# glennhickey/teHmm

Hardware: AMD Instinct MI355X
Metric: genome positions/sec (Viterbi+posterior), 35 states x 10 tracks (higher is better)
Workload: dtype f64

## Files before the change

tehmm_amd/csrc/tehmm_fused.hip.h:

```cpp
#pragma once
#include "tehmm_lane.hip.h"

namespace tehmm {

template <int NT>
struct FusedGeom {
  static constexpr int KS = NT / 4;
  static constexpr int KSP = ((KS + 1) + 1) & ~1;
  static constexpr int RT = (NT + 15) / 16;
  static constexpr int SLICE_B = KSP * 8;
  static constexpr int ROW_D = 4 * KSP;
  static constexpr int ROW_D_LDS = 4 * KSP + 2;
};

#ifndef TEHMM_FUSED_2W
#define TEHMM_FUSED_2W 36
#endif
#define TEHMM_FUSED_BLKW 24
#ifndef TEHMM_FUSED_NSLOT_CAP
#define TEHMM_FUSED_NSLOT_CAP 64
#endif

struct FusedTab {
  const unsigned long long *rixx;
// ... 42 lines not shown
}
__device__ __forceinline__ double item_max4(double t) {
  const unsigned lo = __double2loint(t), hi = __double2hiint(t);
  const auto a = __builtin_amdgcn_permlane32_swap(lo, lo, false, false);
  const auto b = __builtin_amdgcn_permlane32_swap(hi, hi, false, false);
  const double t1 = fmax(__hiloint2double((int)b[0], (int)a[0]), __hiloint2double((int)b[1], (int)a[1]));
  const unsigned lo1 = __double2loint(t1), hi1 = __double2hiint(t1);
  const auto c = __builtin_amdgcn_permlane16_swap(lo1, lo1, false, false);
  const auto d = __builtin_amdgcn_permlane16_swap(hi1, hi1, false, false);
  return fmax(__hiloint2double((int)d[0], (int)c[0]), __hiloint2double((int)d[1], (int)c[1]));
}

typedef unsigned int fused_u4 __attribute__((ext_vector_type(4)));
struct IndexWindow {
  const fused_u4 *src;
  unsigned lds_base;
  int lane, dir, NB;
  int cur = -1;
  fused_u4 r0, r1, r2;
  bool inflight = false;

  __device__ __forceinline__ void request(int blk) {
    if (blk < 0 || blk >= NB) { inflight = false; return; }
    const fused_u4 *p = src + (int64_t)blk * 192 + lane * 3;
    r0 = p[0];
    r1 = p[1];
    r2 = p[2];
    inflight = true;
  }
  __device__ __forceinline__ void commit(int blk) {
    typedef __attribute__((address_space(3))) fused_u4 lds_u4;
    lds_u4 *d = (lds_u4 *)(size_t)(lds_base + (unsigned)((blk & 1) * 3072 + lane * 48));
    d[0] = r0;
    d[1] = r1;
    d[2] = r2;
    cur = blk;
  }
  __device__ __forceinline__ void start(int blk) {
    request(blk);
    commit(blk);
    request(blk + dir);
  }
  __device__ __forceinline__ void need(int blk) {
    if (blk != cur) {
      commit(blk);
      request(blk + dir);
    }
  }
  __device__ __forceinline__ unsigned word_addr(int blk, int r, int FKW, int w) const {
    return lds_base + (unsigned)((blk & 1) * 3072 + ((r * FKW + w) * 16 + (lane & 15)) * 8);
  }
};
__device__ __forceinline__ unsigned long long lds_read_u64(unsigned addr) {
  typedef __attribute__((address_space(3))) const unsigned long long lds_cu64;
  return *(lds_cu64 *)(size_t)addr;
}

template <int NT, bool LOGDOM>
struct EmisStream {
  using G = FusedGeom<NT>;
  static constexpr int NSLOT = G::KS < TEHMM_FUSED_NSLOT_CAP ? G::KS : TEHMM_FUSED_NSLOT_CAP;
  static constexpr int NGS = NSLOT > 1 ? 2 : 1;
  static constexpr int GF = NSLOT >= 8 ? 4 : NSLOT / 2;
  const FusedTab &ft;
  const double *lds;
  IndexWindow &win;
  const int kq;
  unsigned wbase = 0;
  double q[G::KS];
  double sc = 0.0;
  double xa[G::KSP];
  double xc[G::KSP];
  unsigned long long wcur = 0;

  __device__ __forceinline__ EmisStream(const FusedTab &ft_, const double *lds_, IndexWindow &win_, int kq_)
      : ft(ft_), lds(lds_), win(win_), kq(kq_) {}
  static __device__ __forceinline__ int entry(unsigned long long w, int i) { return (int)((w >> (16 * (i & 3))) & 0xffffull); }
  __device__ __forceinline__ unsigned long long word(int w) const { return lds_read_u64(wbase + (unsigned)w * 128u); }
  __device__ __forceinline__ void fold(const double (&x)[G::KSP]) {
#pragma unroll
    for (int s = 0; s < G::KS; ++s) q[s] = LOGDOM ? q[s] + x[s] : q[s] * x[s];
    if (!LOGDOM) sc += x[G::KS];
  }
  __device__ __forceinline__ void glb_request(int i) { fused_load_glb<NT>(ft.ptab, entry(word(i >> 2), i), kq, xa); }
  __device__ __forceinline__ void begin(int e) {
    const int blk = e / ft.SB, r = e - blk * ft.SB;
    win.need(blk);
    wbase = win.word_addr(blk, r, ft.FKW, 0);
#pragma unroll
    for (int s = 0; s < G::KS; ++s) q[s] = LOGDOM ? 0.0 : 1.0;
    sc = 0.0;
    glb_request(0);
    wcur = word(ft.n_glb >> 2);
  }
  __device__ __forceinline__ void slot(int k) {
    if (k >= NSLOT) return;
    const int il = ft.n_glb + k;
    if (k > 0) fold(xc);
    if (k == GF && NSLOT > 1) {
      fold(xa);
      glb_request(1);
    }
    fused_load_lds<NT>(lds, entry(wcur, il), kq, xc);
    if (k + 1 < NSLOT) wcur = word((il + 1) >> 2);
  }
  __device__ __forceinline__ void finish(int N, double (&qo)[G::KS], double &ms) {
    fold(xc);
    fold(xa);
    for (int i = NGS; i < ft.n_glb; ++i) {
      glb_request(i);
      fold(xa);
    }
    for (int il = ft.n_glb + NSLOT; il < ft.K; ++il) {
      fused_load_lds<NT>(lds, entry(word(il >> 2), il), kq, xc);
      fold(xc);
    }
    if (LOGDOM) {
      double m = -INFINITY;
#pragma unroll
      for (int s = 0; s < G::KS; ++s) {
        q[s] *= ft.normalize;
        m = fmax(m, kq + 4 * s < N ? q[s] : -INFINITY);
      }
      m = item_max4(m);
      const bool good = m > -1e20;
#pragma unroll
      for (int s = 0; s < G::KS; ++s) qo[s] = (good && kq + 4 * s < N) ? exp_nonpos(q[s] - m) : 0.0;
      ms = good ? m : 0.0;
    } else {
#pragma unroll
      for (int s = 0; s < G::KS; ++s) qo[s] = q[s];
      ms = sc;
    }
  }
};

template <int NT>
__host__ __device__ inline size_t fused_lds_bytes(int lds_rows, bool post_tiles) {
  return (size_t)lds_rows * FusedGeom<NT>::ROW_D_LDS * 8 + 4 * 2 * 3072 + (post_tiles ? 4 * (16 * NT * 8 + 128) : 0);
}
template <int NT>
__device__ __forceinline__ void fused_stage(const FusedTab &ft, double *lds) {
  const int n = ft.lds_rows * FusedGeom<NT>::ROW_D_LDS;
  for (int i = threadIdx.x; i < n; i += blockDim.x) lds[i] = ft.ptab_lds[i];
}

struct FusedOrder {
  int K, n_glb, FKW, KP, SB, NB, Wu;
  int zero_glb, zero_lds;
  unsigned char order[TEHMM_MAX_TRACKS];
  int base[TEHMM_MAX_TRACKS];
  int cnt[TEHMM_MAX_TRACKS];
};
__global__ __launch_bounds__(256) void k_fused_rowindex(IntervalTab iv, LaneGeom lg, FusedOrder fo, const uint8_t *obs,
                                                        unsigned long long *rixx) {
  const int E = fo.NB * fo.SB;
  const int64_t n = (int64_t)lg.n_groups * 4 * E * 16;
  const int per_blk = 16 * fo.SB;
  for (int64_t idx = blockIdx.x * (int64_t)blockDim.x + threadIdx.x; idx < n; idx += (int64_t)gridDim.x * blockDim.x) {
    const int64_t tb = idx / per_blk;
    const int rem = (int)(idx - tb * per_blk);
    const int i16 = rem / fo.SB;
    const int e = (int)(tb % fo.NB) * fo.SB + (rem - i16 * fo.SB);
    const int64_t tile = tb / fo.NB;
    const int64_t item = tile * 16 + i16;
    const bool valid = item < lg.n_items;
    const int id = valid ? lg.item_iv[item] : 0;
    const int64_t T = iv.len[id];
    int64_t t = (valid ? lg.item_t0[item] : 0) - fo.Wu + e;
    t = t < 0 ? 0 : (t >= T ? T - 1 : t);
    const uint8_t *orow = obs + (iv.pos0[id] + (T > 0 ? t : 0)) * fo.KP;
    const int blk = e / fo.SB, r = e - blk * fo.SB;
    unsigned long long *dst = rixx + ((tile * fo.NB + blk) * TEHMM_FUSED_BLKW + (int64_t)r * fo.FKW) * 16 + i16;
    for (int w = 0; w < fo.FKW; ++w) {
      unsigned long long word = 0;
      for (int b = 0; b < 4; ++b) {
        const int i = 4 * w + b;
        int v = 0;
        if (i < fo.K) {
          const int sym = orow[fo.order[i]];
          v = sym < fo.cnt[i] ? fo.base[i] + sym : (i < fo.n_glb ? fo.zero_glb : fo.zero_lds);
        }
        word |= (unsigned long long)(v & 0xffff) << (16 * b);
      }
      dst[(int64_t)w * 16] = word;
    }
  }
}

template <int NT, bool LOGDOM>
__global__ __launch_bounds__(256) __attribute__((amdgpu_waves_per_eu(NT <= TEHMM_FUSED_2W ? 2 : 1, NT <= TEHMM_FUSED_2W ? 2 : 1)))
void k_fused_fwd(IntervalTab iv, FusedTab ft, LaneGeom lg, int N, int CS, int Wu,
                 const double *__restrict__ tab , float *al32, double *chkf, double *pre,
                 double *end, double *slog32) {
  using G = FusedGeom<NT>;
  constexpr int KS = G::KS, RT = G::RT;
  extern __shared__ double fused_lds[];
  fused_stage<NT>(ft, fused_lds);
  __syncthreads();
  const int lane = threadIdx.x & 63;
  const int tile = blockIdx.x * 4 + (threadIdx.x >> 6);
  if (tile >= lg.n_groups * 4) return;
  const int L = lg.L;
  const int kq = lane >> 4;
  const int64_t item = (int64_t)tile * 16 + (lane & 15);
  const bool valid = item < lg.n_items;
  const int id = valid ? lg.item_iv[item] : 0;
  const int64_t t0 = valid ? lg.item_t0[item] : 0;
  const int64_t T = iv.len[id];
  const int64_t ct0 = (t0 / CS) * CS;
  const bool run = valid && ct0 + CS <= T && ct0 > 0;
  if (!__any(run)) return;
  double tf[RT][KS];
#pragma unroll
  for (int rt = 0; rt < RT; ++rt) {
#pragma unroll
    for (int s = 0; s < KS; ++s) {
      const int j = 16 * rt + (lane & 15), k = 4 * s + kq;
      tf[rt][s] = (j < NT) ? tab[k * NT + j] : 0.0;
    }
  }
  double v[KS];
#pragma unroll
  for (int s = 0; s < KS; ++s) v[s] = (kq + 4 * s < N) ? 1.0 / (double)N : 0.0;
  double slog = 0.0;
  auto vec_out = [&](double *dst) {
    const int64_t po = ((((item >> 6) * NT) + kq) << 6) + (item & 63);
#pragma unroll
    for (int s = 0; s < KS; ++s) dst[po + ((int64_t)(4 * s) << 6)] = v[s];
  };
  const double qnan = __longlong_as_double(0x7ff8000000000000LL);
  IndexWindow win;
  win.src = (const fused_u4 *)ft.rixx + (int64_t)tile * ft.NB * 192;
  win.lds_base = (unsigned)(size_t)(__attribute__((address_space(3))) const double *)fused_lds +
                 (unsigned)(ft.lds_rows * G::ROW_D_LDS * 8 + (threadIdx.x >> 6) * 2 * 3072);
  win.lane = lane;
  win.dir = 1;
  win.NB = ft.NB;
  win.start(0);
  double q[KS], ms;
  EmisStream<NT, LOGDOM> es(ft, fused_lds, win, kq);
  es.begin(0);
#pragma unroll
  for (int k = 0; k < KS; ++k) es.slot(k);
  es.finish(N, q, ms);
  const int E1 = ft.NB * ft.SB - 1;
  es.begin(min(1, E1));
  {
    float2 *ar = (float2 *)al32 + al32_index<NT>(lg, item, 0, kq) / 2;
#pragma unroll
    for (int p = 0; p < (KS + 1) / 2; ++p) ar[(int64_t)p * 64] = make_float2(0.f, 0.f);
  }
#ifdef TEHMM_STAMPS
  unsigned long long stq[4] = {0, 0, 0, 0}, stt = stamp_now();
#define FST(i) do { const unsigned long long n_ = stamp_now(); stq[i] += n_ - stt; stt = n_; } while (0)
#else
#define FST(i)
#endif
  for (int s = -Wu; s < L; ++s) {
    if (s == 0) {
      if (run) vec_out(pre);
      slog = 0.0;
    }
    FST(3);
    lane_d4 acc[RT];
#pragma unroll
    for (int rt = 0; rt < RT; ++rt) acc[rt] = (lane_d4){0.0, 0.0, 0.0, 0.0};
#pragma unroll
    for (int k = 0; k < KS; ++k) {
#pragma unroll
      for (int rt = 0; rt < RT; ++rt) acc[rt] = __builtin_amdgcn_mfma_f64_16x16x4f64(tf[rt][k], v[k], acc[rt], 0, 0, 0);
      es.slot(k);
      __builtin_amdgcn_sched_barrier(0);
    }
    FST(0);
    double qn[KS], msn = 0.0;
    es.finish(N, qn, msn);
    FST(1);
    double a[KS];
    double t = 0.0;
#pragma unroll
    for (int k = 0; k < KS; ++k) {
      a[k] = acc[k >> 2][k & 3] * q[k];
      t += a[k];
    }
    t = item_sum4(t);
    const int e = ((__double2hiint(t) >> 20) & 0x7ff) - 1022;
    const bool okrow = t > 1e-280 && t < INFINITY;
    const double scale = okrow ? __hiloint2double((1023 - e) << 20, 0) : qnan;
#pragma unroll
    for (int k = 0; k < KS; ++k) v[k] = a[k] * scale;
    slog += (double)e * 0.6931471805599453 + ms;
#pragma unroll
    for (int k = 0; k < KS; ++k) q[k] = qn[k];
    const double ms_now = ms;
    ms = msn;
    (void)ms_now;
    es.begin(min(s + 2 + Wu, E1));
    FST(2);
    {
      float2 *ar = (float2 *)al32 + al32_index<NT>(lg, item, s < 0 ? 0 : s, kq) / 2;
#pragma unroll
      for (int p = 0; p < (KS + 1) / 2; ++p)
        ar[(int64_t)p * 64] = run ? make_float2((float)v[2 * p], 2 * p + 1 < KS ? (float)v[2 * p + 1] : 0.f)
                                  : make_float2(0.f, 0.f);
    }
    if (s >= 0 && run) {
      if ((s & 31) == 31) {
        if (kq == 0) slog32[item * (L / 32) + (s >> 5)] = slog;
        if ((s & 63) == 31) {
          double *cr = chkf + (item * (L / 64) + (s >> 6)) * NT + kq;
#pragma unroll
          for (int k = 0; k < KS; ++k) cr[4 * k] = v[k];
        }
      }
    }
  }
  if (run) vec_out(end);
#ifdef TEHMM_STAMPS
  if (lane == 0 && blockIdx.x < 4096)
    for (int i = 0; i < 4; ++i) g_stamps[(blockIdx.x * 4 + (threadIdx.x >> 6)) * 4 + i] = stq[i];
#endif
#undef FST
}

template <int NT, bool LOGDOM, bool EPS, bool ESTEP = false>
__global__ __launch_bounds__(256) __attribute__((amdgpu_waves_per_eu(NT <= TEHMM_FUSED_2W ? 2 : 1, NT <= TEHMM_FUSED_2W ? 2 : 1)))
void k_fused_bwd(IntervalTab iv, FusedTab ft, LaneGeom lg, int N, int CS, int Wu,
                 const double *__restrict__ tab , const float *__restrict__ al32,
                 double *post, double *pre, double *end, double *chk, float *gam32 = nullptr, float *wz32 = nullptr,
                 double *sink = nullptr ) {
  using G = FusedGeom<NT>;
  constexpr int KS = G::KS, RT = G::RT;
  extern __shared__ double fused_lds[];
  fused_stage<NT>(ft, fused_lds);
  __syncthreads();
  const int lane = threadIdx.x & 63;
  const int tile = blockIdx.x * 4 + (threadIdx.x >> 6);
  if (tile >= lg.n_groups * 4) return;
// ... 201 lines not shown
```

tehmm_amd/csrc/tehmm_hip.hip:

```cpp
#include <climits>
#include "tehmm_kernels.hip.h"
#include "tehmm_coop.hip.h"
#include "tehmm_lane.hip.h"
#include "tehmm_lane3.hip.h"
#include "tehmm_place.hip.h"
#include "tehmm_aux.hip.h"
#include "tehmm_fused.hip.h"
#include "tehmm_estep.hip.h"
#include "tehmm_wide_estep.hip.h"
#include "tehmm_wide.hip.h"
#include "tehmm_large.hip.h"
#include "tehmm_map.hip.h"

#include <algorithm>
#include <atomic>
#include <cmath>
#include <cstdio>
#include <cstdlib>
#include <cstring>
#include <mutex>
#include <numeric>
#include <string>
#include <thread>
#include <vector>
// ... 1555 lines not shown
  return TEHMM_OK;
}

template <int NT>
static void launch_vit_stitch(tehmm_batch *b, const tehmm_model *m, const IntervalTab &iv, const VitChunks &vc,
                              hipStream_t st) {
  LaneWork &lw = b->lw;
  hipLaunchKernelGGL((k_vit_stitch<NT>), dim3((vc.n + 3) / 4), dim3(256), 0, st, iv, lane_geom(lw), vc,
                     lane_vit_items(lw), m->N, lw.soft_ties);
  hipLaunchKernelGGL((k_vit_links<NT>), dim3((vc.n + 3) / 4), dim3(256), 0, st, iv, lane_geom(lw), vc,
                     lane_vit_items(lw), m->N);
  hipLaunchKernelGGL(k_vit_runs, dim3(std::max(1, b->n)), dim3(64), 0, st, vc, b->n);
}

static LaneGeom lane_geom(const LaneWork &lw) {
  LaneGeom lg;
  lg.item_iv = lw.item_iv.p; lg.item_t0 = lw.item_t0.p; lg.ifirst = lw.ifirst.p;
  lg.n_items = lw.n_items; lg.n_groups = lw.n_groups; lg.L = lw.L;
  return lg;
}

template <int NT>
static void launch_emis_lane(tehmm_batch *b, const tehmm_model *m, const IntervalTab &iv, const EmisTab &em,
                             bool want_log, bool want_lin, bool want_f32, hipStream_t st) {
  LaneWork &lw = b->lw;
  const size_t lds = (size_t)em.lds_rows * NT * sizeof(double);
  allow_lds(k_emis_lane<NT>, lds);
  hipLaunchKernelGGL((k_emis_lane<NT>), dim3((lw.n_groups + 3) / 4), dim3(256), lds, st, iv, em, lane_geom(lw),
                     m->N, want_log ? lw.B.p : (double *)nullptr, want_lin ? lw.BH.p : (double *)nullptr, lw.MS.p,
                     want_f32 ? lw.B32.p : (float *)nullptr);
}

template <int NT>
static void launch_emis_gain_lane(tehmm_batch *b, const tehmm_model *m, const IntervalTab &iv, const EmisTab &em,
                                  int CS, int Wu, bool ratio, int emis_split, hipStream_t st) {
  LaneWork &lw = b->lw;
  if constexpr (NT >= 12) {
    const bool split = emis_split >= 0 ? emis_split != 0 : lw.n_groups < 2048;
    if (split) {
      constexpr int NW = TEHMM_P2_NW, NU = 2;
      const size_t lds3 = Emis3Geom<NT, NW, NU>::lds_bytes(em.lds_rows);
      const dim3 grid3((lw.n_groups + NU - 1) / NU);
      if constexpr (NT <= TEHMM_RATIO_LANE_MAX) if (ratio) {
        allow_lds(k_emis_gain_lane3<NT, NW, NU, true>, lds3);
        hipLaunchKernelGGL((k_emis_gain_lane3<NT, NW, NU, true>), grid3, dim3(64 * NW * NU), lds3, st, iv, em, lane_geom(lw),
                           m->N, CS, Wu, (const float *)m->ltP.p, lw.B.p, lw.vgain.p, (const double *)b->ratios.p);
        return;
      }
      allow_lds(k_emis_gain_lane3<NT, NW, NU, false>, lds3);
      hipLaunchKernelGGL((k_emis_gain_lane3<NT, NW, NU, false>), grid3, dim3(64 * NW * NU), lds3, st, iv, em, lane_geom(lw),
                         m->N, CS, Wu, (const float *)m->ltP.p, lw.B.p, lw.vgain.p, (const double *)nullptr);
      return;
    }
  }
  const size_t lds = (size_t)em.lds_rows * NT * sizeof(double);
  if constexpr (NT <= TEHMM_RATIO_LANE_MAX) if (ratio) {
    allow_lds(k_emis_gain_lane<NT, true>, lds);
    hipLaunchKernelGGL((k_emis_gain_lane<NT, true>), dim3((lw.n_groups + 3) / 4), dim3(256), lds, st, iv, em,
                       lane_geom(lw), m->N, CS, Wu, (const float *)m->ltP.p, lw.B.p, lw.vgain.p,
                       (const double *)b->ratios.p);
    return;
  }
  allow_lds(k_emis_gain_lane<NT>, lds);
  hipLaunchKernelGGL((k_emis_gain_lane<NT>), dim3((lw.n_groups + 3) / 4), dim3(256), lds, st, iv, em, lane_geom(lw),
                     m->N, CS, Wu, (const float *)m->ltP.p, lw.B.p, lw.vgain.p, (const double *)nullptr);
}

template <int NT>
static void launch_gain_lane(tehmm_batch *b, const tehmm_model *m, const IntervalTab &iv, int CS, int Wu,
                             hipStream_t st) {
  LaneWork &lw = b->lw;
  hipLaunchKernelGGL((k_vit_gain_lane<NT>), dim3((lw.n_groups + 3) / 4), dim3(256), 0, st, iv, lane_geom(lw), m->N,
                     CS, Wu, (const float *)m->ltP.p, (const float *)lw.B32.p, lw.vgain.p);
}

template <int NT>
static void launch_fb_lane(tehmm_batch *b, const tehmm_model *m, const IntervalTab &iv, const EmisTab &em_in,
                           const FbChunks &fc, int Wu, hipStream_t st, hipEvent_t ev_mid) {
  LaneWork &lw = b->lw;
  const LaneGeom lg = lane_geom(lw);
  const dim3 grid((lw.n_groups + 3) / 4);
  const dim3 gridc((fc.n + 255) / 256);
  const dim3 gridit((lw.n_items + 255) / 256);
  const dim3 gridi(std::max(1, b->n));
  const EmisTab em = b->n > 256 ? without_lds_tables(em_in) : em_in;
  size_t lds = ((size_t)2 * 64 * (NT + 1) + 2 * 64 + NT + (size_t)em.lds_rows * NT + 8) * sizeof(double);
  allow_lds(k_fb_fix<NT, 0, false, true>, lds);
  allow_lds(k_fb_fix<NT, 1, false, true>, lds);
  hipStream_t sS = b->sB;
  hipLaunchKernelGGL((k_fb_lane<NT, 0>), grid, dim3(256), 0, st, iv, lg, m->N, fc.CS, Wu, m->AG.p, lw.BH.p,
                     lw.MS.p, lw.AL.p, lw.pre_f.p, lw.end_f.p, lw.slog32.p);
  (void)hipEventRecord(b->evX[0], st);
  (void)hipStreamWaitEvent(sS, b->evX[0], 0);
  hipLaunchKernelGGL((k_fb_itemlinks<NT>), gridit, dim3(256), 0, sS, lg, m->N, lw.pre_f.p, lw.end_f.p, lw.pre_b.p,
                     lw.end_b.p, lw.dl_f.p, lw.lr_f.p, lw.dl_b.p, 1);
  hipLaunchKernelGGL((k_fb_stitch<NT>), gridc, dim3(256), 0, sS, iv, lg, fc, m->N, lw.slog32.p, lw.end_b.p,
                     lw.dl_f.p, lw.lr_f.p, lw.dl_b.p, lw.ok_f.p, lw.ok_b.p, 1);
  hipLaunchKernelGGL(k_fb_runs, gridi, dim3(64), 0, sS, iv, fc, (const int *)lw.ok_f.p, (const int *)lw.ok_b.p,
                     1);
  hipLaunchKernelGGL((k_fb_fix<NT, 0, false, true>), dim3(b->n), dim3(128), lds, sS, iv, em, fc, m->N, m->A.p,
                     m->lt.p, m->pi.p, (const double *)nullptr, lw.AL.p, b->fwd_lp.p, b->dead.p,
                     (double *)nullptr, (int *)nullptr, 1, b->sw.stats.p, lg, (const int *)lw.ok_f.p);
  (void)hipEventRecord(b->evX[1], sS);
  hipLaunchKernelGGL((k_fb_lane<NT, 1>), grid, dim3(256), 0, st, iv, lg, m->N, fc.CS, Wu, m->ATG.p, lw.BH.p,
                     lw.MS.p, lw.BE.p, lw.pre_b.p, lw.end_b.p, (double *)nullptr);
  hipLaunchKernelGGL((k_fb_itemlinks<NT>), gridit, dim3(256), 0, st, lg, m->N, lw.pre_f.p, lw.end_f.p, lw.pre_b.p,
                     lw.end_b.p, lw.dl_f.p, lw.lr_f.p, lw.dl_b.p, 2);
  hipLaunchKernelGGL((k_fb_stitch<NT>), gridc, dim3(256), 0, st, iv, lg, fc, m->N, lw.slog32.p, lw.end_b.p,
                     lw.dl_f.p, lw.lr_f.p, lw.dl_b.p, lw.ok_f.p, lw.ok_b.p, 2);
  hipLaunchKernelGGL(k_fb_runs, gridi, dim3(64), 0, st, iv, fc, (const int *)lw.ok_f.p, (const int *)lw.ok_b.p,
                     2);
  (void)hipEventRecord(ev_mid, st);
  hipLaunchKernelGGL((k_fb_fix<NT, 1, false, true>), dim3(b->n), dim3(128), lds, st, iv, em, fc, m->N, m->A.p,
                     m->lt.p, m->pi.p, (const double *)nullptr, lw.BE.p, b->fwd_lp.p, b->dead.p,
                     (double *)nullptr, (int *)nullptr, 1, b->sw.stats.p, lg, (const int *)lw.ok_b.p);
  (void)hipStreamWaitEvent(st, b->evX[1], 0);
}

template <int NT>
static int fused_prepare(tehmm_batch *b, const tehmm_model *m, const IntervalTab &iv, int Wu, hipStream_t st, FusedOrder &fo) {
  LaneWork &lw = b->lw;
  const LaneGeom lg = lane_geom(lw);
  std::memset(&fo, 0, sizeof(fo));
  fo.K = m->K;
  fo.KP = b->KP;
  fo.Wu = Wu;
  fo.zero_glb = m->R;
  fo.zero_lds = m->lds_zero;
  {
    constexpr int NSLOT = EmisStream<NT, false>::NSLOT, NGS = EmisStream<NT, false>::NGS;
    int slot = 0;
    auto pad = [&]() { fo.order[slot] = 0; fo.base[slot] = 0; fo.cnt[slot] = 0; ++slot; };
    for (int k = 0; k < m->K; ++k)
      if (m->ldsbase[k] < 0) { fo.order[slot] = (unsigned char)k; fo.base[slot] = m->rowbase[k]; fo.cnt[slot] = m->rowcnt[k]; ++slot; }
    while (slot < NGS) pad();
    fo.n_glb = slot;
    for (int k = 0; k < m->K; ++k)
      if (m->ldsbase[k] >= 0) { fo.order[slot] = (unsigned char)k; fo.base[slot] = m->ldsbase[k]; fo.cnt[slot] = m->rowcnt[k]; ++slot; }
    while (slot - fo.n_glb < NSLOT) pad();
    fo.K = slot;
  }
  {
    static const int ok[] = {1, 2, 3, 4, 6, 8, 12, 24};
    int need = (fo.K + 3) / 4;
    fo.FKW = 24;
    for (int d : ok) if (d >= need) { fo.FKW = d; break; }
  }
  fo.SB = TEHMM_FUSED_BLKW / fo.FKW;
  fo.NB = (lw.L + 2 * Wu + fo.SB - 1) / fo.SB;
  if (!lw.rix.p || lw.rix_model != m->uid || lw.rix_L != lw.L || lw.rix_Wu != Wu) {
    const size_t words = (size_t)lw.n_groups * 4 * fo.NB * TEHMM_FUSED_BLKW * 16;
    lw.rix_model = 0;
    HIPCHK(lw.rix.ensure(words + 16));
    hipLaunchKernelGGL(k_fused_rowindex, dim3(grid_for((int64_t)lw.n_groups * 4 * fo.NB * fo.SB * 16, 256, 1 << 20)),
                       dim3(256), 0, st, iv, lg, fo, (const uint8_t *)b->obs.p, lw.rix.p);
    lw.rix_model = m->uid;
    lw.rix_L = lw.L;
    lw.rix_Wu = Wu;
  }
  return TEHMM_OK;
}

template <int NT>
static int launch_fused_fb(tehmm_batch *b, const tehmm_model *m, const IntervalTab &iv, const EmisTab &em_in,
                           const FbChunks &fc, int Wu, hipStream_t st, hipEvent_t ev_fwd, hipEvent_t ev_mid,
                           bool estep = false, int half = 0, hipEvent_t ev_fwdk = nullptr) {
  LaneWork &lw = b->lw;
  const LaneGeom lg = lane_geom(lw);
  const dim3 gridm((unsigned)lw.n_groups);
  const dim3 gridc((fc.n + 255) / 256);
  const dim3 gridit((lw.n_items + 255) / 256);
  const dim3 gridi(std::max(1, b->n));
  FusedOrder fo;
  if (int rcp = fused_prepare<NT>(b, m, iv, Wu, st, fo)) return rcp;
  FusedTab ft;
  ft.rixx = lw.rix.p;
  ft.ptab = m->ptab.p;
  ft.ptab_lds = m->ptab_lds.p;
  ft.FKW = fo.FKW;
  ft.SB = fo.SB;
  ft.NB = fo.NB;
  ft.K = fo.K;
  ft.n_glb = fo.n_glb;
  ft.lds_rows = m->lds_rows;
  ft.normalize = m->normalize;
  const EmisTab emc = b->n > 256 ? without_lds_tables(em_in) : em_in;
  const size_t lds_f = fused_lds_bytes<NT>(m->lds_rows, false), lds_b = fused_lds_bytes<NT>(m->lds_rows, true);
  const size_t lds_c = ((size_t)2 * 64 * (NT + 1) + 2 * 64 + NT + (size_t)emc.lds_rows * NT + 8) * sizeof(double);
  allow_lds(k_fb_fix<NT, 0, false, true, true>, lds_c);
  allow_lds(k_fb_fix<NT, 1, false, true, true>, lds_c);
#define TEHMM_FUSED_LAUNCH(LOG_)                                                                                     \
  do {                                                                                                              \
    allow_lds(k_fused_fwd<NT, LOG_>, lds_f);                                                                         \
    allow_lds(k_fused_bwd<NT, LOG_, true>, lds_b);                                                                   \
    if (half != 2) {                                                                                                \
    hipLaunchKernelGGL((k_fused_fwd<NT, LOG_>), gridm, dim3(256), lds_f, st, iv, ft, lg, m->N, fc.CS, Wu,            \
                       (const double *)m->A.p, lw.AL32.p, lw.chkf.p, lw.pre_f.p, lw.end_f.p, lw.slog32.p);           \
    if (ev_fwdk) (void)hipEventRecord(ev_fwdk, st);                                                                  \
    hipLaunchKernelGGL((k_fb_itemlinks<NT>), gridit, dim3(256), 0, st, lg, m->N, lw.pre_f.p, lw.end_f.p,             \
                       lw.pre_b.p, lw.end_b.p, lw.dl_f.p, lw.lr_f.p, lw.dl_b.p, 1);                                  \
    hipLaunchKernelGGL((k_fb_stitch<NT>), gridc, dim3(256), 0, st, iv, lg, fc, m->N, lw.slog32.p, lw.end_b.p,        \
                       lw.dl_f.p, lw.lr_f.p, lw.dl_b.p, lw.ok_f.p, lw.ok_b.p, 1);                                    \
    hipLaunchKernelGGL(k_fb_runs, gridi, dim3(64), 0, st, iv, fc, (const int *)lw.ok_f.p, (const int *)lw.ok_b.p, 1); \
    hipLaunchKernelGGL((k_fb_fix<NT, 0, false, true, true>), dim3(b->n), dim3(128), lds_c, st, iv, emc, fc, m->N,    \
                       m->A.p, m->lt.p, m->pi.p, (const double *)nullptr, (double *)nullptr, b->fwd_lp.p, b->dead.p, \
                       (double *)nullptr, (int *)nullptr, 1, b->sw.stats.p, lg, (const int *)lw.ok_f.p,              \
                       (const double *)lw.chkf.p, (double *)nullptr, lw.AL32.p, (const double *)lw.end_f.p);         \
    (void)hipEventRecord(ev_fwd, st);                                                                                \
    }                                                                                                               \
    if (half == 1) break;                                                                                           \
    if (estep) {                                                                                                    \
      allow_lds(k_fused_bwd<NT, LOG_, false, true>, lds_f);                                                          \
      hipLaunchKernelGGL((k_fused_bwd<NT, LOG_, false, true>), gridm, dim3(256), lds_f, st, iv, ft, lg, m->N, fc.CS, \
                         Wu, (const double *)m->A.p, (const float *)lw.AL32.p, (double *)nullptr, lw.pre_b.p,        \
                         lw.end_b.p, lw.chk.p, lw.GAM32.p, lw.WZ32.p);                                               \
    } else {                                                                                                        \
      hipLaunchKernelGGL((k_fused_bwd<NT, LOG_, true>), gridm, dim3(256), lds_b, st, iv, ft, lg, m->N, fc.CS,         \
                         Wu, (const double *)m->A.p, (const float *)lw.AL32.p, b->post.p, lw.pre_b.p, lw.end_b.p,    \
                         lw.chk.p, (float *)nullptr, (float *)nullptr, lw.sink.p);                                   \
    }                                                                                                               \
  } while (0)
  if (m->ptab_log) TEHMM_FUSED_LAUNCH(true);
  else TEHMM_FUSED_LAUNCH(false);
#undef TEHMM_FUSED_LAUNCH
  if (half == 1) {
    HIPCHK(hipGetLastError());
    return TEHMM_OK;
  }
  hipLaunchKernelGGL((k_fb_itemlinks<NT>), gridit, dim3(256), 0, st, lg, m->N, lw.pre_f.p, lw.end_f.p, lw.pre_b.p,
                     lw.end_b.p, lw.dl_f.p, lw.lr_f.p, lw.dl_b.p, 2);
  hipLaunchKernelGGL((k_fb_stitch<NT>), gridc, dim3(256), 0, st, iv, lg, fc, m->N, lw.slog32.p, lw.end_b.p,
                     lw.dl_f.p, lw.lr_f.p, lw.dl_b.p, lw.ok_f.p, lw.ok_b.p, 2);
  hipLaunchKernelGGL(k_fb_runs, gridi, dim3(64), 0, st, iv, fc, (const int *)lw.ok_f.p, (const int *)lw.ok_b.p,
                     2);
  (void)hipEventRecord(ev_mid, st);
  if (estep) {
    const size_t lds_e = lds_c + (size_t)64 * (NT + 1) * sizeof(double);
    allow_lds(k_fb_fix<NT, 1, false, true, true, true>, lds_e);
    hipLaunchKernelGGL((k_fb_fix<NT, 1, false, true, true, true>), dim3(b->n), dim3(128), lds_e, st, iv, emc, fc, m->N,
                       m->A.p, m->lt.p, m->pi.p, (const double *)nullptr, (double *)nullptr, b->fwd_lp.p, b->dead.p,
                       (double *)nullptr, (int *)nullptr, 1, b->sw.stats.p, lg, (const int *)lw.ok_b.p,
                       (const double *)lw.chk.p, (double *)nullptr, lw.AL32.p, (const double *)nullptr, lw.GAM32.p,
                       lw.WZ32.p);
    return TEHMM_OK;
  }
  hipLaunchKernelGGL((k_fb_fix<NT, 1, false, true, true>), dim3(b->n), dim3(128), lds_c, st, iv, emc, fc, m->N, m->A.p,
                     m->lt.p, m->pi.p, (const double *)nullptr, (double *)nullptr, b->fwd_lp.p, b->dead.p,
                     (double *)nullptr, (int *)nullptr, 1, b->sw.stats.p, lg, (const int *)lw.ok_b.p,
                     (const double *)lw.chk.p, b->post.p, lw.AL32.p, (const double *)nullptr);
  return TEHMM_OK;
}

template <int NT>
static void launch_combine_lane(tehmm_batch *b, const tehmm_model *m, const IntervalTab &iv, hipStream_t st) {
  LaneWork &lw = b->lw;
  hipLaunchKernelGGL((k_combine_lane<NT, true>), dim3((unsigned)lw.n_groups * (lw.L / 8)), dim3(256), 0, st, iv,
                     lane_geom(lw), m->N, lw.AL.p, lw.BE.p, b->post.p);
}

template <int NT>
static void launch_fb_spec(tehmm_batch *b, const tehmm_model *m, const IntervalTab &iv, const EmisTab &em,
                           const FbChunks &fc, hipStream_t st) {
  size_t lds = ((size_t)4 * 64 * (NT + 1) + 4 * 64) * sizeof(double);
  const int grid = std::min((fc.n + 3) / 4, 4096);
  allow_lds(k_fb_spec<NT, 0>, lds);
  allow_lds(k_fb_spec<NT, 1>, lds);
  hipLaunchKernelGGL((k_fb_spec<NT, 0>), dim3(grid), dim3(256), lds, st, iv, em, fc, m->N, m->A.p, b->post.p);
  hipLaunchKernelGGL((k_fb_spec<NT, 1>), dim3(grid), dim3(256), lds, st, iv, em, fc, m->N, m->A.p, b->beta.p);
}

template <int NT>
static void launch_fb_fix(tehmm_batch *b, const tehmm_model *m, const IntervalTab &iv, const EmisTab &em_in,
                          const FbChunks &fc, hipStream_t sF, hipStream_t sBk) {
  const EmisTab em = b->n > 256 ? without_lds_tables(em_in) : em_in;
  size_t lds = ((size_t)2 * 64 * (NT + 1) + 2 * 64 + NT + (size_t)em.lds_rows * NT + 8) * sizeof(double);
  allow_lds(k_fb_fix<NT, 0, false, false>, lds);
  allow_lds(k_fb_fix<NT, 1, false, false>, lds);
  hipLaunchKernelGGL((k_fb_fix<NT, 0, false, false>), dim3(b->n), dim3(128), lds, sF, iv, em, fc, m->N, m->A.p,
                     m->lt.p, m->pi.p, (const double *)nullptr, b->post.p, b->fwd_lp.p, b->dead.p,
                     (double *)nullptr, (int *)nullptr, 1, b->sw.stats.p, LaneGeom(), (const int *)nullptr);
  hipLaunchKernelGGL((k_fb_fix<NT, 1, false, false>), dim3(b->n), dim3(128), lds, sBk, iv, em, fc, m->N, m->A.p,
                     m->lt.p, m->pi.p, (const double *)nullptr, b->beta.p, b->fwd_lp.p, b->dead.p,
                     (double *)nullptr, (int *)nullptr, 1, b->sw.stats.p, LaneGeom(), (const int *)nullptr);
}

template <int... NTs, class F>
static void nt_dispatch_of(int NP, F &&f) {
  (void)((NP == NTs && (f(std::integral_constant<int, NTs>{}), true)) || ...);
}
template <class F>
static void nt_dispatch(int NP, F &&f) {
#ifdef TEHMM_DEV_NT
  nt_dispatch_of<TEHMM_DEV_NT>(NP, f);
#else
  nt_dispatch_of<4, 8, 12, 16, 20, 24, 28, 32, 36, 40, 48, 56, 64>(NP, f);
#endif
}



template <int NPW>
static void launch_wide_passes(tehmm_batch *b, const tehmm_model *m, const IntervalTab &iv, const LaneGeom &lg, int Wu,
                               hipStream_t st, hipEvent_t mid) {
  WideWork &w = b->ww;
  const size_t lds = WideGeom<NPW>::FRAG_BYTES;
  allow_lds(k_wide_fwd<NPW>, lds);
  allow_lds(k_wide_bwd<NPW>, lds);
  const dim3 grid((unsigned)std::max(1, w.n_groups));
// ... 2466 lines not shown
```

Before: 1.534 billion.

## Restructure row-index build with wave-cooperative LDS staging and coalesced vector stores

Rewrites the observation-to-row-index kernel so each wavefront owns a tile and a run of blocks. It loads the raw observation rows with coalesced 32-bit reads into LDS, prefetching the next block, then builds the packed index words from LDS and writes them as 128-bit vector stores. The slot table is staged in shared memory, and FKW becomes a template parameter dispatched by a switch. This targets the per-thread byte gathers and strided 64-bit stores of the old grid-stride loop. The cost is extra LDS, wave barriers, and a new failure case when the observation row is wider than an index record.

```diff
diff --git a/tehmm_amd/csrc/tehmm_fused.hip.h b/tehmm_amd/csrc/tehmm_fused.hip.h
--- a/tehmm_amd/csrc/tehmm_fused.hip.h
+++ b/tehmm_amd/csrc/tehmm_fused.hip.h
@@ -218,39 +218,111 @@
   int base[TEHMM_MAX_TRACKS];
   int cnt[TEHMM_MAX_TRACKS];
 };
+#define TEHMM_RIX_ND ((16 * TEHMM_FUSED_BLKW + 63) / 64)
+__device__ __forceinline__ void rix_wave_sync() {
+  __builtin_amdgcn_fence(__ATOMIC_RELEASE, "wavefront");
+  __builtin_amdgcn_wave_barrier();
+  __builtin_amdgcn_fence(__ATOMIC_ACQUIRE, "wavefront");
+}
+template <int FKW>
 __global__ __launch_bounds__(256) void k_fused_rowindex(IntervalTab iv, LaneGeom lg, FusedOrder fo, const uint8_t *obs,
-                                                        unsigned long long *rixx) {
-  const int E = fo.NB * fo.SB;
-  const int64_t n = (int64_t)lg.n_groups * 4 * E * 16;
-  const int per_blk = 16 * fo.SB;
-  for (int64_t idx = blockIdx.x * (int64_t)blockDim.x + threadIdx.x; idx < n; idx += (int64_t)gridDim.x * blockDim.x) {
-    const int64_t tb = idx / per_blk;
-    const int rem = (int)(idx - tb * per_blk);
-    const int i16 = rem / fo.SB;
-    const int e = (int)(tb % fo.NB) * fo.SB + (rem - i16 * fo.SB);
-    const int64_t tile = tb / fo.NB;
+                                                        unsigned long long *rixx, int NBC) {
+  static_assert(TEHMM_FUSED_BLKW % FKW == 0, "FKW must divide the block");
+  constexpr int SB = TEHMM_FUSED_BLKW / FKW;
+  constexpr int ND = TEHMM_RIX_ND;
+  __shared__ uint2 slot_tab[4 * FKW];
+  __shared__ uint32_t rows_lds[4][16 * TEHMM_FUSED_BLKW];
+  if (threadIdx.x < 4 * FKW) {
+    const int i = threadIdx.x;
+    uint2 s = make_uint2(0u, 0u);
+    if (i < fo.K) {
+      s.x = (unsigned)fo.order[i] | ((unsigned)fo.cnt[i] << 8);
+      s.y = ((unsigned)fo.base[i] & 0xffffu) | (((unsigned)(i < fo.n_glb ? fo.zero_glb : fo.zero_lds) & 0xffffu) << 16);
+    }
+    slot_tab[i] = s;
+  }
+  __syncthreads();
+  const int lane = threadIdx.x & 63, wv = __builtin_amdgcn_readfirstlane(threadIdx.x >> 6);
+  const int n_run = (fo.NB + NBC - 1) / NBC;
+  const int64_t unit = (int64_t)blockIdx.x * 4 + wv;
+  const int64_t tile = unit / n_run;
+  if (tile >= (int64_t)lg.n_groups * 4) return;
+  const int b0 = (int)(unit - tile * n_run) * NBC, b1 = min(b0 + NBC, fo.NB);
+  uint32_t *rows = rows_lds[wv];
+  const int kp4 = fo.KP >> 2, nd = SB * kp4;
+  const int nk = (16 * nd + 63) >> 6;
+  int64_t src_off[ND];
+  int ulo[ND], uhi[ND], urow[ND], lds_at[ND];
+#pragma unroll
+  for (int k = 0; k < ND; ++k) {
+    if (k >= nk) break;
+    const int g = min(lane + 64 * k, 16 * nd - 1);
+    const int i16 = g / nd;
+    const int j = g - i16 * nd;
+    lds_at[k] = g;
+    urow[k] = j / kp4;
+    const int col = j - urow[k] * kp4;
     const int64_t item = tile * 16 + i16;
     const bool valid = item < lg.n_items;
     const int id = valid ? lg.item_iv[item] : 0;
+    const int64_t t0 = valid ? lg.item_t0[item] : 0;
     const int64_t T = iv.len[id];
-    int64_t t = (valid ? lg.item_t0[item] : 0) - fo.Wu + e;
-    t = t < 0 ? 0 : (t >= T ? T - 1 : t);
-    const uint8_t *orow = obs + (iv.pos0[id] + (T > 0 ? t : 0)) * fo.KP;
-    const int blk = e / fo.SB, r = e - blk * fo.SB;
-    unsigned long long *dst = rixx + ((tile * fo.NB + blk) * TEHMM_FUSED_BLKW + (int64_t)r * fo.FKW) * 16 + i16;
-    for (int w = 0; w < fo.FKW; ++w) {
-      unsigned long long word = 0;
-      for (int b = 0; b < 4; ++b) {
-        const int i = 4 * w + b;
-        int v = 0;
-        if (i < fo.K) {
-          const int sym = orow[fo.order[i]];
-          v = sym < fo.cnt[i] ? fo.base[i] + sym : (i < fo.n_glb ? fo.zero_glb : fo.zero_lds);
+    int64_t lo = max((int64_t)fo.Wu - t0, (int64_t)0), hi = T - 1 - t0 + fo.Wu;
+    if (T <= 0) lo = hi = fo.Wu - t0;
+    ulo[k] = (int)lo;
+    uhi[k] = (int)min(hi, (int64_t)fo.NB * SB);
+    src_off[k] = (iv.pos0[id] + t0 - fo.Wu) * fo.KP + col * 4;
+  }
+  unsigned sym_at[3][4], cnt[3][4], rbase[3][4], rzero[3][4];
+#pragma unroll
+  for (int k = 0; k < 3; ++k) {
+    const int rw = (lane >> 3) + 8 * k, r = rw / FKW, w = rw - r * FKW;
+    const unsigned row_at = (unsigned)((2 * (lane & 7) * SB + r) * fo.KP);
+#pragma unroll
+    for (int b = 0; b < 4; ++b) {
+      const uint2 s = slot_tab[4 * w + b];
+      sym_at[k][b] = row_at + (s.x & 0xffu);
+      cnt[k][b] = s.x >> 8;
+      rbase[k][b] = s.y & 0xffffu;
+      rzero[k][b] = s.y >> 16;
+    }
+  }
+  const unsigned item_stride = (unsigned)(SB * fo.KP);
+  const uint8_t *rowb = (const uint8_t *)rows;
+  auto fetch = [&](int blk, uint32_t (&v)[ND]) {
+#pragma unroll
+    for (int k = 0; k < ND; ++k) {
+      if (k >= nk) break;
+      const int e = min(max(blk * SB + urow[k], ulo[k]), uhi[k]);
+      v[k] = *(const uint32_t *)(obs + (src_off[k] + (int64_t)e * fo.KP));
+    }
+  };
+  uint32_t v[ND];
+  fetch(b0, v);
+  for (int blk = b0; blk < b1; ++blk) {
+#pragma unroll
+    for (int k = 0; k < ND; ++k) {
+      if (k >= nk) break;
+      rows[lds_at[k]] = v[k];
+    }
+    rix_wave_sync();
+    if (blk + 1 < b1) fetch(blk + 1, v);
+    fused_u4 *dst = (fused_u4 *)(rixx + (tile * fo.NB + blk) * (int64_t)(TEHMM_FUSED_BLKW * 16));
+#pragma unroll
+    for (int k = 0; k < 3; ++k) {
+      unsigned out[2][2] = {{0u, 0u}, {0u, 0u}};
+#pragma unroll
+      for (int it = 0; it < 2; ++it) {
+#pragma unroll
+        for (int b = 0; b < 4; ++b) {
+          const unsigned sym = rowb[sym_at[k][b] + it * item_stride];
+          const unsigned x = sym < cnt[k][b] ? (rbase[k][b] + sym) & 0xffffu : rzero[k][b];
+          out[it][b >> 1] |= x << (16 * (b & 1));
         }
-        word |= (unsigned long long)(v & 0xffff) << (16 * b);
-      }
-      dst[(int64_t)w * 16] = word;
-    }
+      }
+      dst[lane + 64 * k] = (fused_u4){out[0][0], out[0][1], out[1][0], out[1][1]};
+    }
+    rix_wave_sync();
   }
 }
 
diff --git a/tehmm_amd/csrc/tehmm_hip.hip b/tehmm_amd/csrc/tehmm_hip.hip
--- a/tehmm_amd/csrc/tehmm_hip.hip
+++ b/tehmm_amd/csrc/tehmm_hip.hip
@@ -1731,8 +1731,21 @@
     const size_t words = (size_t)lw.n_groups * 4 * fo.NB * TEHMM_FUSED_BLKW * 16;
     lw.rix_model = 0;
     HIPCHK(lw.rix.ensure(words + 16));
-    hipLaunchKernelGGL(k_fused_rowindex, dim3(grid_for((int64_t)lw.n_groups * 4 * fo.NB * fo.SB * 16, 256, 1 << 20)),
-                       dim3(256), 0, st, iv, lg, fo, (const uint8_t *)b->obs.p, lw.rix.p);
+    if (fo.KP / 4 > fo.FKW) return fail(TEHMM_ERR_UNSUPPORTED, "fused_prepare: observation row wider than an index record");
+    const int64_t tiles = (int64_t)lw.n_groups * 4;
+    const int nbc = tiles >= 1024 ? 8 : 2;
+    const int64_t units = tiles * ((fo.NB + nbc - 1) / nbc);
+    const dim3 grid((unsigned)((units + 3) / 4));
+    switch (fo.FKW) {
+#define TEHMM_RIX_CASE(W_)                                                                                      \
+      case W_:                                                                                                  \
+        hipLaunchKernelGGL(k_fused_rowindex<W_>, grid, dim3(256), 0, st, iv, lg, fo, (const uint8_t *)b->obs.p, \
+                           lw.rix.p, nbc);                                                                      \
+        break;
+      TEHMM_RIX_CASE(1) TEHMM_RIX_CASE(2) TEHMM_RIX_CASE(3) TEHMM_RIX_CASE(4)
+      TEHMM_RIX_CASE(6) TEHMM_RIX_CASE(8) TEHMM_RIX_CASE(12) TEHMM_RIX_CASE(24)
+#undef TEHMM_RIX_CASE
+    }
     lw.rix_model = m->uid;
     lw.rix_L = lw.L;
     lw.rix_Wu = Wu;
```

Result: no change. 1.546 billion (median of 6 runs) (+0.8%).
